# VCISwang/STCD

Measured on AMD Instinct MI355X. Metric: image-pairs/sec (256x256 bf16 SiamUnet_diff train), higher is better.
Workload: dtype bf16; 1 GPU; SiamUnet_diff(3,2) 256x256 full training step (fwd + cross_entropy + bwd + AdamW), 16 pairs/GPU, synthetic LEVIR-CD-shaped pairs resident in HBM; global_batch=16, image=256, parallelism=dp1

## Files before the change

stcd_amd/csrc/common.h:

```cpp
#pragma once
#include <hip/hip_runtime.h>
#include <stdint.h>
#include <stdio.h>
#include <string>
#include <string.h>

#include "../../include/stcd_hip.h"

namespace stcd {

typedef __bf16 bf16;

enum DType { F32 = STCD_DTYPE_F32, BF16 = STCD_DTYPE_BF16 };
inline size_t dsize(int dt) { return dt == BF16 ? 2 : 4; }

void set_error(const std::string& msg);

#define STCD_CHECK(cond, msg)                                              \
    do {                                                                   \
        if (!(cond)) {                                                     \
            ::stcd::set_error(std::string(__func__) + ": " + (msg));       \
            return 1;                                                      \
        }                                                                  \
    } while (0)
// ... 226 lines not shown
int launch_conv_halo(const stcd_conv_geom& g, const ConvMfmaPlan& p, const ConvHaloPlan& hp, const void* in, const void* wf,
                     const float* bias, void* out, hipStream_t s, const ConvEpi* epi = nullptr);

struct ConvDmaPlan {
    int tiles_m = 0, tiles_n = 0, blocks = 0, lds_bytes = 0;
    bool ok = false;
};
ConvDmaPlan conv_dma_plan(const stcd_conv_geom& g, const ConvMfmaPlan& p);
int launch_conv_dma(const stcd_conv_geom& g, const ConvMfmaPlan& p, const ConvDmaPlan& dp, const void* in, const void* wf,
                    const float* bias, void* out, hipStream_t s, const ConvEpi* epi = nullptr);

bool conv_small_ok(const stcd_conv_geom& g, const ConvMfmaPlan& p);
int conv_small_blocks(const stcd_conv_geom& g, int groups);
int launch_conv_small(const stcd_conv_geom& g, const void* in, const void* wf_modeB, const float* bias, void* out,
                      bool out_nchw_f32, int groups, long long* stat_acc, int cpad, hipStream_t s, const XfSrc* xf = nullptr,
                      const BwdSum* bs = nullptr);
bool conv_small_bwdsum_ok(const stcd_conv_geom& g);
struct WgradMfmaPlan {
    int WCI = 1, NTW = 1, gx = 1, gy = 1, gz = 1;
    int64_t slab_floats = 0;
    int wi_valid = 0;
    int gemm = 0;
    int dma = 0;
    bool ok = false;
};
WgradMfmaPlan wgrad_mfma_plan(const stcd_conv_geom& g, int kpad, int wld, bool allow_wide = false, int force_co64 = -1);
int launch_wgrad_mfma(const stcd_conv_geom& g, const WgradMfmaPlan& p, const void* in, const void* dout, float* slab,
                      int kpad, int wld, hipStream_t s);
struct WgradJob {
    stcd_conv_geom g;
    int64_t in_off, dout_off, slab_off;
    int kpad, wld;
    int dymin, dxmin, HH, HWp;
    int tiles_x, tiles_y, ntiles;
    int xrow_bytes;
    int x_bytes, y_bytes;
    int co_valid;
    unsigned in_bytes, dout_bytes;
    int gx, gy, gz;
    int start;
    int lds_bytes;
    int wi_valid;
    int dma_L, dma_nk;
    int pad_;
    int64_t xf_stat_off, xf_mask_off;
    int xf_C, xf_groups, xf_npg, pad2_;
};
WgradMfmaPlan wgrad_gemm_plan(const stcd_conv_geom& g, int kpad, int wld);
WgradJob wgrad_gemm_make_job(const stcd_conv_geom& g, const WgradMfmaPlan& p, int64_t in_off, int64_t dout_off, int64_t slab_off,
                             int kpad, int wld);
int launch_wgrad_gemm_group(int W, const WgradJob* jobs_dev, int njobs, int total_blocks, const char* base, hipStream_t s);
WgradMfmaPlan wgrad_dma_plan(const stcd_conv_geom& g, int kpad, int wld);
void wgrad_dma_set_split(WgradMfmaPlan& p, const stcd_conv_geom& g, int S, int kpad, int wld);
WgradJob wgrad_dma_make_job(const stcd_conv_geom& g, const WgradMfmaPlan& p, int64_t in_off, int64_t dout_off, int64_t slab_off,
                            int kpad, int wld);
int launch_wgrad_dma_group(const WgradJob* jobs_dev, int njobs, int total_blocks, const char* base, hipStream_t s);
WgradJob wgrad_make_job(const stcd_conv_geom& g, const WgradMfmaPlan& p, int64_t in_off, int64_t dout_off, int64_t slab_off,
                        int kpad, int wld);
void wgrad_job_set_xf(WgradJob& a, int64_t stat_off, int64_t mask_off, int C, int groups, int npg);
int wgrad_variant_slots(int WCI, int NTW, bool t9, int lds_bytes);
int launch_wgrad_group(int WCI, int NTW, bool t9, const WgradJob* jobs_dev, int njobs, int total_blocks, int lds_bytes,
                       const char* base, hipStream_t s, bool xf = false);
struct PackSpec;
struct ReduceJob {
    int64_t start, count;
    int64_t slab_off;
    int64_t out_off;
    int64_t slab_stride;
    int gx, ntaps, K, N, kpad, wld;
    int ks, kn_major;
    int8_t ky[9], kx[9];
    int8_t tiled, parts, pad_[4];
};
void launch_reduce_jobs(const ReduceJob* jobs_dev, int njobs, int64_t total, const char* ws, float* grads, hipStream_t s);
void launch_reduce_dw(const float* slab, int gx, const stcd_conv_geom& g, int K, int N, int kpad, int wld,
                      const PackSpec* ps, float* out, hipStream_t s);

struct PackSpec {
    int ks;
// ... 227 lines not shown
```

stcd_amd/csrc/engine.hip:

```cpp
#include <algorithm>
#include <climits>
#include <cstdint>
#include <array>
#include <cstring>
#include <memory>
#include <vector>

#include "common.h"

namespace stcd {

static thread_local std::string g_err;
void set_error(const std::string& msg) { g_err = msg; }

enum ConvKind { K_CONV3 = 0, K_CONVT3_S1 = 1, K_UPCONV = 2, K_CONV1 = 3, K_CONVT2 = 4, K_CONV3_S2 = 5, K_CONV1_S2 = 6, K_STEM7 = 7 };

struct TRef { int64_t off = -1; int ld = 0; };
struct GRef { int64_t off = -1; int ld = 0; int64_t goff = 0; };

static inline int round8(int c) { return (c + 7) & ~7; }

struct ConvW {
    std::string name;
    int kind = 0, cin = 0, cout = 0;
// ... 23 lines not shown
    ConvDmaPlan dma;
    ConvHaloPlan halo;
};
struct WgradOp {
    stcd_conv_geom g{};
    int conv = -1, tap0 = 0, kreal = 0, nreal = 0;
    WgradMfmaPlan plan;
    int64_t slab = -1;
    int stage = 0;
    int64_t in_off = -1, dout_off = -1;
    bool grouped = false;
    int group = -1;
    int64_t xf_stat_off = -1, xf_mask_off = -1; int xf_C = 0, xf_groups = 1, xf_npg = 1;
    bool tail = false;
    bool own_taps = false;
    int8_t oky[9] = {0}, okx[9] = {0};
};
struct WgradGroup {
    int WCI = 1, NTW = 1; bool t9 = false;
    bool xf = false;
    bool tail = false;
    int gemm = 0;
    int dma = 0;
    std::vector<WgradJob> jobs;
    int total_blocks = 0, lds_bytes = 0;
    int64_t table_off = -1;
    double flops = 0.0, bytes = 0.0;
    int seen = 0; bool launched = false;
};

struct Cbrd {
    ConvOp fwd, dgr; WgradOp wg;
    int conv = -1, bn = -1, drop = -1;
    int N = 0, H = 0, W = 0, groups = 1, npg = 0;
    TRef in; int K = 0;
    TRef Y; GRef A; TRef P; TRef dPool; bool pool = false;
    GRef dA; TRef dY; TRef dIn; bool has_dIn = false;
    int64_t stat = -1;
    int64_t facc = -1, bacc = -1;
    const Cbrd* dgr_bwd = nullptr;
    bool bwd_sums_fused = false;
    int64_t dgr_sum_acc = -1; int dgr_sum_c0 = 0, dgr_sum_C = 0;
    TRef fuse_dst;
    bool virt = false; const Cbrd* xsrc = nullptr;
};
struct XConc {
// ... 393 lines not shown
    g.ntaps = t;
    static const int start[4] = {0, 1, 3, 5};
    *tap0 = start[py * 2 + px];
    return g;
}

static void conv_work(const stcd_engine& e, const stcd_conv_geom& g, int kreal, int nreal, double* flops, double* bytes);

static void pick_gemm_or_res(const stcd_engine& e, ConvOp& op, const stcd_conv_geom& g, int groups) {
    op.gemm = ConvGemmPlan();
    if (!e.use_gemm || op.small) return;
    static const int env_mode = [] { const char* v = getenv("STCD_GEMM_OVER_RES"); return v ? atoi(v) : -1; }();
    const int mode = env_mode >= 0 ? env_mode : (e.cf ? 1 : 0);
    if (op.res.ok && !(mode == 2 || (mode == 1 && op.res.NT == 1))) return;
    op.gemm = conv_gemm_plan(g, op.plan, groups);
    if (op.gemm.ok) op.res = ConvResPlan();
    static const bool halo_on = [] { const char* v = getenv("STCD_HALO_KERNEL"); return v && v[0] == '1'; }();
    op.halo = ConvHaloPlan();
    op.dma = ConvDmaPlan();
    if (op.gemm.ok && (int64_t)g.n * g.hm * g.wm >= 256 * 192) op.dma = conv_dma_plan(g, op.plan);
    if (halo_on && op.gemm.ok && (int64_t)g.n * ((g.hm + 15) / 16) * ((g.wm + 15) / 16) >= 512) op.halo = conv_halo_plan(g, op.plan);
}

static WgradMfmaPlan pick_wgrad_plan(const stcd_engine& e, const stcd_conv_geom& g, int kpad, int wld) {
    if (e.use_gemm && e.use_wgroup && 2.0 * g.n * g.hm * g.wm * (double)g.ci * g.co >= 0.8e9) {
        WgradMfmaPlan p = wgrad_gemm_plan(g, kpad, wld);
        if (p.ok) return p;
    }
    if (e.use_wgroup && (g.ntaps == 9 || (e.cf && g.ntaps == 4)) && (int64_t)g.n * g.hm * g.wm >= 65536) {
        WgradMfmaPlan p = wgrad_dma_plan(g, kpad, wld);
        if (p.ok) return p;
    }
    return wgrad_mfma_plan(g, kpad, wld, is_snunet(e.arch) || (e.cf && g.ntaps == 9));
}

static void build_pack_jobs(stcd_engine& e, Bump& ws) {
    for (int st = 0; st < 2; ++st) { e.rjobs[st].clear(); e.rjobs_total[st] = 0; }
    for (int st = 0; st < 2; ++st) e.wgroups[st].clear();
    if (e.dt == BF16 && e.use_mfma) {
        if (e.use_wgroup) {
            for (WgradOp* op : e.wgrad_ops) {
                if (!op->plan.ok) continue;
                const bool t9 = !op->plan.dma && op->g.ntaps == 9;
                std::vector<WgradGroup>& gs = e.wgroups[op->stage];
                size_t gi = 0;
                for (; gi < gs.size(); ++gi)
                    if (gs[gi].gemm == op->plan.gemm && gs[gi].dma == op->plan.dma && gs[gi].WCI == op->plan.WCI && gs[gi].NTW == op->plan.NTW && gs[gi].t9 == t9 && gs[gi].xf == (op->xf_C > 0) && gs[gi].tail == op->tail) break;
                if (gi == gs.size()) { WgradGroup g; g.WCI = op->plan.WCI; g.NTW = op->plan.NTW; g.t9 = t9; g.gemm = op->plan.gemm; g.dma = op->plan.dma; g.xf = op->xf_C > 0; g.tail = op->tail; gs.push_back(g); }
                op->grouped = true;
            }
            for (int st = 0; st < 2; ++st)
                for (WgradGroup& G : e.wgroups[st]) {
                    if (G.gemm) { G.lds_bytes = 2 * 2 * G.gemm * (64 * 64 + 8 * 32); continue; }
                    if (G.dma) {
                        G.lds_bytes = 128 * 1024;
                        std::vector<WgradOp*> dops;
                        for (WgradOp* op : e.wgrad_ops)
                            if (op->grouped && op->stage == st && op->plan.dma) dops.push_back(op);
                        auto blocks_at = [&](int64_t kt) {
                            int64_t b = 0;
                            for (WgradOp* op : dops) {
                                const int64_t M = (int64_t)op->g.n * op->g.hi * op->g.wi;
                                b += ((M + kt * 64 - 1) / (kt * 64)) * op->plan.gy * op->plan.gz;
                            }
                            return b;
                        };
                        int64_t lo = 1, hi = 1;
                        static const int dma_env = [] { const char* v = getenv("STCD_WGRAD_DMA_BLOCKS"); return v && atoi(v) > 0 ? atoi(v) : 0; }();
                        static const bool cf_side_env = [] { const char* v = getenv("STCD_CF_SIDE"); return !(v && v[0] == '0'); }();
                        const int dma_blocks = dma_env ? dma_env : (e.wg_side_on && cf_side_env ? 192 : 256);
                        while (blocks_at(hi) > dma_blocks) hi *= 2;
                        while (lo < hi) { const int64_t mid = (lo + hi) / 2; if (blocks_at(mid) <= dma_blocks) hi = mid; else lo = mid + 1; }
                        for (WgradOp* op : dops) {
                            const ConvW& cv = e.convs[op->conv];
                            const int64_t M = (int64_t)op->g.n * op->g.hi * op->g.wi;
                            int64_t S = (M + lo * 64 - 1) / (lo * 64);
                            const int64_t slab_bytes = (int64_t)op->g.ntaps * cv.fwd.kpad * cv.fwd.wld * 4;
                            S = std::min<int64_t>(S, std::max<int64_t>(1, ((int64_t)64 << 20) / slab_bytes));
                            wgrad_dma_set_split(op->plan, op->g, (int)S, cv.fwd.kpad, cv.fwd.wld);
                        }
                        continue;
                    }
                    std::vector<WgradOp*> ops;
                    int64_t W = 0;
                    for (WgradOp* op : e.wgrad_ops)
                        if (op->grouped && op->stage == st && !op->plan.gemm && !op->plan.dma && op->plan.WCI == G.WCI && op->plan.NTW == G.NTW && (op->g.ntaps == 9) == G.t9 && (op->xf_C > 0) == G.xf && op->tail == G.tail) {
                            ops.push_back(op);
                            const int64_t ntiles = (int64_t)op->g.n * ((op->g.wm + 15) / 16) * ((op->g.hm + 7) / 8);
                            W += ntiles * op->plan.gy * op->plan.gz;
                        }
                    for (WgradOp* op : ops) {
                        const ConvW& cv = e.convs[op->conv];
                        WgradJob j = wgrad_make_job(op->g, op->plan, 0, 0, 0, cv.fwd.kpad, cv.fwd.wld);
                        if (op->xf_C > 0) wgrad_job_set_xf(j, op->xf_stat_off, op->xf_mask_off, op->xf_C, op->xf_groups, op->xf_npg);
                        G.lds_bytes = std::max(G.lds_bytes, j.lds_bytes);
                    }
                    int slots = wgrad_variant_slots(G.WCI, G.NTW, G.t9, G.lds_bytes);
                    if (st == 0 && e.wg_side_on && e.wg_side_div > 1 && fc_family(e)) slots = std::max(64, slots / e.wg_side_div);
                    const int64_t rounds = e.wgroup_rounds;
                    const int64_t tpb = std::max<int64_t>(e.wgroup_min_tiles, (W + rounds * slots - 1) / (rounds * slots));
                    for (WgradOp* op : ops) {
                        const ConvW& cv = e.convs[op->conv];
                        const int64_t ntiles = (int64_t)op->g.n * ((op->g.wm + 15) / 16) * ((op->g.hm + 7) / 8);
                        const int64_t slab_bytes = (int64_t)op->g.ntaps * cv.fwd.kpad * cv.fwd.wld * 4;
                        int64_t gx = std::max<int64_t>(1, (ntiles + tpb - 1) / tpb);
                        gx = std::min<int64_t>(gx, std::max<int64_t>(1, ((int64_t)32 << 20) / slab_bytes));
                        op->plan.gx = (int)gx;
                        op->plan.slab_floats = gx * op->g.ntaps * cv.fwd.kpad * cv.fwd.wld;
                    }
                }
        }
        int64_t cur[2] = {0, 0};
        for (WgradOp* op : e.wgrad_ops) {
            if (!op->plan.ok) continue;
            const ConvW& cv = e.convs[op->conv];
            op->slab = ws.take(op->plan.slab_floats * 4);
            if (op->grouped) {
                const bool t9 = !op->plan.dma && op->g.ntaps == 9;
                for (WgradGroup& G : e.wgroups[op->stage])
                    if (G.gemm == op->plan.gemm && G.dma == op->plan.dma && G.WCI == op->plan.WCI && G.NTW == op->plan.NTW && G.t9 == t9 && G.xf == (op->xf_C > 0) && G.tail == op->tail) {
                        op->group = (int)(&G - e.wgroups[op->stage].data());
                        WgradJob j = op->plan.dma ? wgrad_dma_make_job(op->g, op->plan, op->in_off, op->dout_off, op->slab, cv.fwd.kpad, cv.fwd.wld)
                                   : op->plan.gemm ? wgrad_gemm_make_job(op->g, op->plan, op->in_off, op->dout_off, op->slab, cv.fwd.kpad, cv.fwd.wld)
                                                   : wgrad_make_job(op->g, op->plan, op->in_off, op->dout_off, op->slab, cv.fwd.kpad, cv.fwd.wld);
                        if (op->xf_C > 0 && !op->plan.dma && !op->plan.gemm) wgrad_job_set_xf(j, op->xf_stat_off, op->xf_mask_off, op->xf_C, op->xf_groups, op->xf_npg);
                        j.start = G.total_blocks;
                        G.total_blocks += j.gx * j.gy * j.gz;
                        G.jobs.push_back(j);
                        double fl, by;
                        conv_work(e, op->g, op->kreal, op->nreal, &fl, &by);
                        G.flops += fl; G.bytes += by;
                    }
            }
            ReduceJob j{};
            j.slab_off = op->slab; j.out_off = cv.w_off;
            j.slab_stride = (int64_t)op->g.ntaps * cv.fwd.kpad * cv.fwd.wld;
            j.gx = op->plan.gx; j.ntaps = op->g.ntaps; j.K = cv.cin; j.N = cv.cout; j.kpad = cv.fwd.kpad; j.wld = cv.fwd.wld;
            j.ks = cv.fwd.ks; j.kn_major = cv.fwd.kn_major;
            for (int t = 0; t < op->g.ntaps; ++t) {
                j.ky[t] = op->own_taps ? op->oky[t] : cv.fwd.ky[op->tap0 + t];
                j.kx[t] = op->own_taps ? op->okx[t] : cv.fwd.kx[op->tap0 + t];
            }
            j.tiled = (int64_t)j.ntaps * j.K * j.N >= 512 * 1024;
            if (!j.tiled) {
                const int64_t outs = (int64_t)j.ntaps * j.K * j.N;
                int parts = 1;
                while (parts < 64 && parts * 32 < j.gx) parts *= 2;
                j.parts = (int8_t)parts;
// ... 292 lines not shown
                   (P.groups == 1 || P.dA.goff == (int64_t)P.npg * P.H * P.W * P.dA.ld);
        };
        auto scan = [&](std::vector<Cbrd>& v) {
            for (size_t i = 1; i < v.size(); ++i) {
                Cbrd& N = v[i]; Cbrd& P = v[i - 1];
                if (N.has_dIn && N.dgr_sum_acc < 0 && dest_ok(P, N.dgr, N.dIn.off, N.dIn.ld, N.N)) { N.dgr_bwd = &P; P.bwd_sums_fused = true; }
            }
        };
        scan(e.enc); scan(e.dec);
        if (!e.dec.empty() && dest_ok(e.dec.back(), e.final_dgr, e.dFinalIn.off, e.dFinalIn.ld, e.dec.back().N)) {
            e.final_dgr_bwd = &e.dec.back(); e.dec.back().bwd_sums_fused = true;
        }
    }

    e.final_xsrc = nullptr; e.fc_virt_layers = 0;
    for (auto& L : e.enc) { L.virt = false; L.xsrc = nullptr; }
    for (auto& L : e.dec) { L.virt = false; L.xsrc = nullptr; }
    if (e.use_virt && e.dt == BF16 && e.use_mfma && e.use_wgroup && !fc_cross(e)) {
        auto fwd_ok = [&](const ConvOp& op, bool nchw) {
            if (op.wf < 0 || (op.gemm.ok && !nchw)) return false;
            if (op.small && e.use_small) return true;
            return op.res.ok && !nchw && !op.res.single_halo;
        };
        auto wg_ok = [&](const WgradOp& op) { return op.plan.ok && !op.plan.gemm && !op.plan.dma && op.plan.WCI < 4 && op.plan.NTW < 4; };
        auto link = [&](Cbrd& P, ConvOp& cf, WgradOp& cw, bool nchw) {
            if (P.pool || P.fuse_dst.off >= 0) return false;
            if (!fwd_ok(cf, nchw) || !wg_ok(cw)) return false;
            P.virt = true; ++e.fc_virt_layers;
            cw.in_off = P.Y.off;
            cw.xf_stat_off = P.stat;
            cw.xf_mask_off = (P.drop >= 0) ? e.masks + e.drops[P.drop].off * 4 : -1;
            cw.xf_C = e.convs[P.conv].cout; cw.xf_groups = P.groups; cw.xf_npg = P.npg;
            return true;
        };
        for (size_t i = 0; i + 1 < e.enc.size(); ++i) {
            Cbrd& P = e.enc[i]; Cbrd& Cn = e.enc[i + 1];
            if (Cn.in.off != P.A.off) continue;
            if (link(P, Cn.fwd, Cn.wg, false)) { Cn.xsrc = &P; Cn.in.off = P.Y.off; Cn.in.ld = P.Y.ld; }
        }
        for (size_t i = 0; i < e.dec.size(); ++i) {
            Cbrd& P = e.dec[i];
            if (i + 1 < e.dec.size() && e.dec[i + 1].in.off == P.A.off) {
                Cbrd& Cn = e.dec[i + 1];
                if (link(P, Cn.fwd, Cn.wg, false)) { Cn.xsrc = &P; Cn.in.off = P.Y.off; Cn.in.ld = P.Y.ld; }
            } else if (e.finalIn.off == P.A.off) {
                if (link(P, e.final_fwd, e.final_wg, true)) { e.final_xsrc = &P; e.finalIn.off = P.Y.off; e.finalIn.ld = P.Y.ld; }
            }
        }
    }

// ... 234 lines not shown
                                        hipMemcpyHostToDevice, c.s));
            if (!e.rjobs[k].empty())
                STCD_HIP(hipMemcpyAsync(c.at(e.rjobs_off[k]), e.rjobs[k].data(), e.rjobs[k].size() * sizeof(ReduceJob),
                                        hipMemcpyHostToDevice, c.s));
            for (WgradGroup& G : e.wgroups[k])
                STCD_HIP(hipMemcpyAsync(c.at(G.table_off), G.jobs.data(), G.jobs.size() * sizeof(WgradJob), hipMemcpyHostToDevice, c.s));
        }
        if (!e.bias_jobs.empty())
            STCD_HIP(hipMemcpyAsync(c.at(e.bias_jobs_off), e.bias_jobs.data(), e.bias_jobs.size() * sizeof(BiasJob), hipMemcpyHostToDevice, c.s));
        e.jobs_uploaded_ws = c.ws;
    }
    const int k = with_dgrad ? 1 : 0;
    if (k == 0 && e.weights_tag != 0 && e.weights_tag == e.packed_tag && e.packed_ws == (const void*)c.ws && e.packed_params == (const void*)c.params)
        return 0;
    ProfScope prof(c, PC_PACK, 0.0, 0.0);
    launch_pack_jobs(c.at<PackJob>(e.jobs_off[k]), (int)e.jobs[k].size(), e.jobs_total[k], c.params, c.ws, c.s);
    e.packed_tag = k == 0 ? e.weights_tag : 0; e.packed_ws = c.ws; e.packed_params = c.params; e.packed_level = k;
    return 0;
}

static void launch_wgroup(const Ctx& c, WgradGroup& G) {
    {
        char kname[64];
        if (G.dma) snprintf(kname, sizeof(kname), "k_wgrad_dma");
        else if (G.gemm) snprintf(kname, sizeof(kname), "k_wgrad_gemm<%d>", G.gemm);
        else snprintf(kname, sizeof(kname), "k_wgrad_group<%d, %d, %s>", G.WCI, G.NTW, G.t9 ? "true" : "false");
        ProfScope prof(c, PC_WGRAD, G.flops, G.bytes, kname);
        G.launched = true;
        if (G.dma) {
            launch_wgrad_dma_group(c.at<WgradJob>(G.table_off), (int)G.jobs.size(), G.total_blocks, c.ws, c.s);
            return;
        }
        if (G.gemm) {
            launch_wgrad_gemm_group(G.gemm, c.at<WgradJob>(G.table_off), (int)G.jobs.size(), G.total_blocks, c.ws, c.s);
            return;
        }
        if (launch_wgrad_group(G.WCI, G.NTW, G.t9, c.at<WgradJob>(G.table_off), (int)G.jobs.size(), G.total_blocks, G.lds_bytes,
                               c.ws, c.s, G.xf) != 0)
            set_error("grouped weight-gradient launch exceeds the LDS budget");
    }
}

static void wgroup_member_ready(const Ctx& c, const WgradOp& op) {
    stcd_engine& e = c.e;
    if (op.group < 0 || op.group >= (int)e.wgroups[op.stage].size()) return;
    WgradGroup& G = e.wgroups[op.stage][op.group];
    if (++G.seen < (int)G.jobs.size() || G.launched) return;
    if (e.wg_cur_side) {
        if (hipEventRecord(e.wg_fork, c.s) != hipSuccess || hipStreamWaitEvent(e.wg_cur_side, e.wg_fork, 0) != hipSuccess) { set_error("side-stream fork failed"); return; }
        Ctx cs{e, c.ws, c.params, c.grads, e.wg_cur_side};
        launch_wgroup(cs, G);
// ... 1935 lines not shown
}

static int check_geom(const stcd_conv_geom* g) {
    STCD_CHECK(g != nullptr, "geometry is null");
    STCD_CHECK(g->ntaps >= 1 && g->ntaps <= 9, "ntaps must be in [1,9]");
    STCD_CHECK(g->ci >= 8 && g->ci % 8 == 0 && g->ldi >= g->ci && g->ldi % 8 == 0, "ci/ldi must be multiples of 8");
    STCD_CHECK(g->co >= 1 && g->ldo >= g->co, "bad co/ldo");
    STCD_CHECK(g->in_stride >= 1 && g->out_stride >= 1 && g->n >= 1 && g->hm >= 1 && g->wm >= 1, "bad sizes");
    STCD_CHECK((g->hm - 1) * g->out_stride + g->oy0 < g->ho && (g->wm - 1) * g->out_stride + g->ox0 < g->wo,
               "output positions exceed the output buffer");
    return 0;
}
static int op_dma_splits(const stcd_conv_geom& g, const WgradMfmaPlan& p) {
    const int64_t M = (int64_t)g.n * g.hi * g.wi;
    return (int)std::max<int64_t>(1, std::min<int64_t>(256 / std::max(1, p.gy * p.gz), M / 512));
}
int64_t stcd_op_scratch_bytes(const stcd_conv_geom* g) {
    if (!g) return 0;
    ConvMfmaPlan p = conv_mfma_plan(*g);
    WgradMfmaPlan w = wgrad_mfma_plan(*g, g->ci, g->co), ww = wgrad_mfma_plan(*g, g->ci, g->co, true);
    WgradMfmaPlan wg = wgrad_gemm_plan(*g, g->ci, g->co);
    WgradMfmaPlan wd = wgrad_dma_plan(*g, g->ci, g->co);
    if (wd.ok) wgrad_dma_set_split(wd, *g, op_dma_splits(*g, wd), g->ci, g->co);
    return std::max<int64_t>(p.wf_elems * 2, std::max(std::max(std::max(w.slab_floats, ww.slab_floats), wg.ok ? wg.slab_floats : 0), wd.ok ? wd.slab_floats : 0) * 4) + 1024;
}
int stcd_op_conv(int dtype, int impl, const stcd_conv_geom* g, const void* in, const float* w, const float* bias,
                 void* out, void* scratch, int64_t scratch_bytes, void* hip_stream) {
    if (check_geom(g)) return 1;
    STCD_CHECK(in && w && out, "null pointer argument");
    if (impl == 1 || impl == 2 || impl == 3 || impl == 6) {
        STCD_CHECK(dtype == STCD_DTYPE_BF16, "the MFMA implementation is bf16 only");
        ConvMfmaPlan p = conv_mfma_plan(*g);
        STCD_CHECK(p.ok, "geometry not supported by the MFMA kernel");
        STCD_CHECK(scratch && scratch_bytes >= p.wf_elems * 2, "scratch too small for the fragment-order filter");
        launch_pack_frag(*g, p, w, g->ci, g->co, scratch, (hipStream_t)hip_stream);
        if (impl == 3) {
            const ConvHaloPlan hp = conv_halo_plan(*g, p);
            STCD_CHECK(hp.ok, "geometry not supported by the resident-halo kernel (3x3 stride 1, Ci % 64 == 0, Co % 128 == 0)");
            STCD_CHECK(launch_conv_halo(*g, p, hp, in, scratch, bias, out, (hipStream_t)hip_stream) == 0, "launch failed");
            STCD_HIP(hipGetLastError());
            return 0;
        }
        if (impl == 6) {
            const ConvDmaPlan dp = conv_dma_plan(*g, p);
            STCD_CHECK(dp.ok, "geometry not supported by the LDS-DMA kernel (Ci % 64 == 0, Co % 256 == 0, (Ci / 64) * taps even and >= 4)");
            STCD_CHECK(launch_conv_dma(*g, p, dp, in, scratch, bias, out, (hipStream_t)hip_stream) == 0, "launch failed");
            STCD_HIP(hipGetLastError());
// ... 37 lines not shown
        WgradMfmaPlan p = wgrad_mfma_plan(*g, g->ci, g->co, impl >= 4, impl == 5 ? 1 : 0);
        STCD_CHECK(p.ok, "geometry not supported by the MFMA kernel");
        STCD_CHECK(scratch && scratch_bytes >= p.slab_floats * 4, "scratch too small for the partial slabs");
        STCD_CHECK(launch_wgrad_mfma(*g, p, in, dout, (float*)scratch, g->ci, g->co, (hipStream_t)hip_stream) == 0, "LDS budget exceeded");
        launch_reduce_dw((const float*)scratch, p.gx, *g, g->ci, g->co, g->ci, g->co, nullptr, dw, (hipStream_t)hip_stream);
        STCD_HIP(hipGetLastError());
        return 0;
    }
    if (impl == 7) {
        STCD_CHECK(dtype == STCD_DTYPE_BF16, "the MFMA implementation is bf16 only");
        WgradMfmaPlan p = wgrad_dma_plan(*g, g->ci, g->co);
        STCD_CHECK(p.ok, "geometry not supported by the LDS-DMA weight-gradient kernel (stride 1, full map >= 64 wide, Ci % 256 == 0, Co % 256 == 0)");
        wgrad_dma_set_split(p, *g, op_dma_splits(*g, p), g->ci, g->co);
        const int64_t table = (p.slab_floats * 4 + 255) & ~(int64_t)255;
        STCD_CHECK(scratch && scratch_bytes >= table + (int64_t)sizeof(WgradJob), "scratch too small for the partial slabs + job table");
        WgradJob j = wgrad_dma_make_job(*g, p, (int64_t)(intptr_t)in, (int64_t)(intptr_t)dout, (int64_t)(intptr_t)scratch, g->ci, g->co);
        STCD_HIP(hipMemcpyAsync((char*)scratch + table, &j, sizeof(j), hipMemcpyHostToDevice, (hipStream_t)hip_stream));
        STCD_HIP(hipStreamSynchronize((hipStream_t)hip_stream));
        launch_wgrad_dma_group((const WgradJob*)((char*)scratch + table), 1, p.gx * p.gy * p.gz, nullptr, (hipStream_t)hip_stream);
        launch_reduce_dw((const float*)scratch, p.gx, *g, g->ci, g->co, g->ci, g->co, nullptr, dw, (hipStream_t)hip_stream);
        STCD_HIP(hipGetLastError());
        return 0;
    }
    if (impl == 3) {
        STCD_CHECK(dtype == STCD_DTYPE_BF16, "the MFMA implementation is bf16 only");
        WgradMfmaPlan p = wgrad_gemm_plan(*g, g->ci, g->co);
        STCD_CHECK(p.ok, "geometry not supported by the GEMM weight-gradient kernel (one tap, Ci >= 64, Co >= 64)");
        const int64_t table = (p.slab_floats * 4 + 255) & ~(int64_t)255;
        STCD_CHECK(scratch && scratch_bytes >= table + (int64_t)sizeof(WgradJob), "scratch too small for the partial slabs + job table");
        WgradJob j = wgrad_gemm_make_job(*g, p, (int64_t)(intptr_t)in, (int64_t)(intptr_t)dout, (int64_t)(intptr_t)scratch, g->ci, g->co);
        STCD_HIP(hipMemcpyAsync((char*)scratch + table, &j, sizeof(j), hipMemcpyHostToDevice, (hipStream_t)hip_stream));
        STCD_HIP(hipStreamSynchronize((hipStream_t)hip_stream));
        launch_wgrad_gemm_group(p.gemm, (const WgradJob*)((char*)scratch + table), 1, p.gx * p.gy * p.gz, nullptr, (hipStream_t)hip_stream);
        launch_reduce_dw((const float*)scratch, p.gx, *g, g->ci, g->co, g->ci, g->co, nullptr, dw, (hipStream_t)hip_stream);
        STCD_HIP(hipGetLastError());
        return 0;
    }
    STCD_CHECK(impl == 0, "impl must be 0 (reference FMA), 1 / 4 (MFMA tile kernel, 4: wide tile allowed), 3 (MFMA position-GEMM kernel) or 7 (LDS-DMA kernel)");
    STCD_HIP(hipMemsetAsync(dw, 0, (size_t)g->ntaps * g->ci * g->co * 4, (hipStream_t)hip_stream));
    launch_wgrad_ref(dtype, *g, in, dout, dw, g->ci, g->co, (hipStream_t)hip_stream);
    STCD_HIP(hipGetLastError());
    return 0;
}

}
```

Before: 7772 image-pairs/sec.

## Add row-streaming MFMA weight-gradient kernel for narrow-channel 3x3 convs

Adds a new weight-gradient kernel that streams whole image rows of input and output-gradient through LDS ring buffers with buffer-to-LDS DMA. It computes all nine 3x3 taps from three resident input rows using transposed LDS reads and bf16 MFMA, then reduces partial slabs across blocks. The planner uses it for large-map convs with few channels (Ci 8-32, Co <=32) in the SiamUnet family, splitting a fixed block budget across grouped ops in proportion to their size. The aim is to cut redundant input reloads and the poor MFMA utilisation of the tile kernel on thin channels. In exchange it uses a large LDS footprint with one block per CU, and it falls back to the tile plan when the layer is fused with a virtual forward.

```diff
diff --git a/stcd_amd/csrc/common.h b/stcd_amd/csrc/common.h
--- a/stcd_amd/csrc/common.h
+++ b/stcd_amd/csrc/common.h
@@ -272,6 +272,7 @@
     int wi_valid = 0;
     int gemm = 0;
     int dma = 0;
+    int rows = 0;
     bool ok = false;
 };
 WgradMfmaPlan wgrad_mfma_plan(const stcd_conv_geom& g, int kpad, int wld, bool allow_wide = false, int force_co64 = -1);
@@ -305,6 +306,11 @@
 WgradJob wgrad_dma_make_job(const stcd_conv_geom& g, const WgradMfmaPlan& p, int64_t in_off, int64_t dout_off, int64_t slab_off,
                             int kpad, int wld);
 int launch_wgrad_dma_group(const WgradJob* jobs_dev, int njobs, int total_blocks, const char* base, hipStream_t s);
+WgradMfmaPlan wgrad_rows_plan(const stcd_conv_geom& g, int kpad, int wld, bool force = false);
+void wgrad_rows_set_blocks(WgradMfmaPlan& p, const stcd_conv_geom& g, int blocks, int kpad, int wld);
+WgradJob wgrad_rows_make_job(const stcd_conv_geom& g, const WgradMfmaPlan& p, int64_t in_off, int64_t dout_off, int64_t slab_off,
+                             int kpad, int wld);
+int launch_wgrad_rows_group(const WgradJob* jobs_dev, int njobs, int total_blocks, int lds_bytes, const char* base, hipStream_t s);
 WgradJob wgrad_make_job(const stcd_conv_geom& g, const WgradMfmaPlan& p, int64_t in_off, int64_t dout_off, int64_t slab_off,
                         int kpad, int wld);
 void wgrad_job_set_xf(WgradJob& a, int64_t stat_off, int64_t mask_off, int C, int groups, int npg);
diff --git a/stcd_amd/csrc/engine.hip b/stcd_amd/csrc/engine.hip
--- a/stcd_amd/csrc/engine.hip
+++ b/stcd_amd/csrc/engine.hip
@@ -69,6 +69,7 @@
     bool tail = false;
     int gemm = 0;
     int dma = 0;
+    int rows = 0;
     std::vector<WgradJob> jobs;
     int total_blocks = 0, lds_bytes = 0;
     int64_t table_off = -1;
@@ -508,6 +509,9 @@
     if (halo_on && op.gemm.ok && (int64_t)g.n * ((g.hm + 15) / 16) * ((g.wm + 15) / 16) >= 512) op.halo = conv_halo_plan(g, op.plan);
 }
 
+static WgradMfmaPlan wgrad_tile_plan(const stcd_engine& e, const stcd_conv_geom& g, int kpad, int wld) {
+    return wgrad_mfma_plan(g, kpad, wld, is_snunet(e.arch) || (e.cf && g.ntaps == 9));
+}
 static WgradMfmaPlan pick_wgrad_plan(const stcd_engine& e, const stcd_conv_geom& g, int kpad, int wld) {
     if (e.use_gemm && e.use_wgroup && 2.0 * g.n * g.hm * g.wm * (double)g.ci * g.co >= 0.8e9) {
         WgradMfmaPlan p = wgrad_gemm_plan(g, kpad, wld);
@@ -517,7 +521,11 @@
         WgradMfmaPlan p = wgrad_dma_plan(g, kpad, wld);
         if (p.ok) return p;
     }
-    return wgrad_mfma_plan(g, kpad, wld, is_snunet(e.arch) || (e.cf && g.ntaps == 9));
+    if (e.use_wgroup && e.use_mfma && fc_family(e) && (int64_t)g.n * g.hm * g.wm >= 65536) {
+        WgradMfmaPlan p = wgrad_rows_plan(g, kpad, wld);
+        if (p.ok && p.WCI * p.NTW > 1) return p;
+    }
+    return wgrad_tile_plan(e, g, kpad, wld);
 }
 
 static void build_pack_jobs(stcd_engine& e, Bump& ws) {
@@ -531,8 +539,8 @@
                 std::vector<WgradGroup>& gs = e.wgroups[op->stage];
                 size_t gi = 0;
                 for (; gi < gs.size(); ++gi)
-                    if (gs[gi].gemm == op->plan.gemm && gs[gi].dma == op->plan.dma && gs[gi].WCI == op->plan.WCI && gs[gi].NTW == op->plan.NTW && gs[gi].t9 == t9 && gs[gi].xf == (op->xf_C > 0) && gs[gi].tail == op->tail) break;
-                if (gi == gs.size()) { WgradGroup g; g.WCI = op->plan.WCI; g.NTW = op->plan.NTW; g.t9 = t9; g.gemm = op->plan.gemm; g.dma = op->plan.dma; g.xf = op->xf_C > 0; g.tail = op->tail; gs.push_back(g); }
+                    if (gs[gi].gemm == op->plan.gemm && gs[gi].dma == op->plan.dma && gs[gi].rows == op->plan.rows && gs[gi].WCI == op->plan.WCI && gs[gi].NTW == op->plan.NTW && gs[gi].t9 == t9 && gs[gi].xf == (op->xf_C > 0) && gs[gi].tail == op->tail) break;
+                if (gi == gs.size()) { WgradGroup g; g.WCI = op->plan.WCI; g.NTW = op->plan.NTW; g.t9 = t9; g.gemm = op->plan.gemm; g.dma = op->plan.dma; g.rows = op->plan.rows; g.xf = op->xf_C > 0; g.tail = op->tail; gs.push_back(g); }
                 op->grouped = true;
             }
             for (int st = 0; st < 2; ++st)
@@ -567,10 +575,27 @@
                         }
                         continue;
                     }
+                    if (G.rows) {
+                        std::vector<WgradOp*> rops;
+                        double total = 0.0;
+                        for (WgradOp* op : e.wgrad_ops)
+                            if (op->grouped && op->stage == st && op->plan.rows && op->plan.WCI == G.WCI && op->plan.NTW == G.NTW && op->tail == G.tail) {
+                                rops.push_back(op);
+                                total += (double)op->g.n * op->g.hi * op->g.wi * (op->g.ci + op->g.co);
+                            }
+                        for (WgradOp* op : rops) {
+                            const ConvW& cv = e.convs[op->conv];
+                            const double share = (double)op->g.n * op->g.hi * op->g.wi * (op->g.ci + op->g.co) / total;
+                            wgrad_rows_set_blocks(op->plan, op->g, std::max(1, (int)(256 * share + 0.5)), cv.fwd.kpad, cv.fwd.wld);
+                            const WgradJob j = wgrad_rows_make_job(op->g, op->plan, 0, 0, 0, cv.fwd.kpad, cv.fwd.wld);
+                            G.lds_bytes = std::max(G.lds_bytes, j.lds_bytes);
+                        }
+                        continue;
+                    }
                     std::vector<WgradOp*> ops;
                     int64_t W = 0;
                     for (WgradOp* op : e.wgrad_ops)
-                        if (op->grouped && op->stage == st && !op->plan.gemm && !op->plan.dma && op->plan.WCI == G.WCI && op->plan.NTW == G.NTW && (op->g.ntaps == 9) == G.t9 && (op->xf_C > 0) == G.xf && op->tail == G.tail) {
+                        if (op->grouped && op->stage == st && !op->plan.gemm && !op->plan.dma && !op->plan.rows && op->plan.WCI == G.WCI && op->plan.NTW == G.NTW && (op->g.ntaps == 9) == G.t9 && (op->xf_C > 0) == G.xf && op->tail == G.tail) {
                             ops.push_back(op);
                             const int64_t ntiles = (int64_t)op->g.n * ((op->g.wm + 15) / 16) * ((op->g.hm + 7) / 8);
                             W += ntiles * op->plan.gy * op->plan.gz;
@@ -604,12 +629,13 @@
             if (op->grouped) {
                 const bool t9 = !op->plan.dma && op->g.ntaps == 9;
                 for (WgradGroup& G : e.wgroups[op->stage])
-                    if (G.gemm == op->plan.gemm && G.dma == op->plan.dma && G.WCI == op->plan.WCI && G.NTW == op->plan.NTW && G.t9 == t9 && G.xf == (op->xf_C > 0) && G.tail == op->tail) {
+                    if (G.gemm == op->plan.gemm && G.dma == op->plan.dma && G.rows == op->plan.rows && G.WCI == op->plan.WCI && G.NTW == op->plan.NTW && G.t9 == t9 && G.xf == (op->xf_C > 0) && G.tail == op->tail) {
                         op->group = (int)(&G - e.wgroups[op->stage].data());
-                        WgradJob j = op->plan.dma ? wgrad_dma_make_job(op->g, op->plan, op->in_off, op->dout_off, op->slab, cv.fwd.kpad, cv.fwd.wld)
+                        WgradJob j = op->plan.rows ? wgrad_rows_make_job(op->g, op->plan, op->in_off, op->dout_off, op->slab, cv.fwd.kpad, cv.fwd.wld)
+                                   : op->plan.dma ? wgrad_dma_make_job(op->g, op->plan, op->in_off, op->dout_off, op->slab, cv.fwd.kpad, cv.fwd.wld)
                                    : op->plan.gemm ? wgrad_gemm_make_job(op->g, op->plan, op->in_off, op->dout_off, op->slab, cv.fwd.kpad, cv.fwd.wld)
                                                    : wgrad_make_job(op->g, op->plan, op->in_off, op->dout_off, op->slab, cv.fwd.kpad, cv.fwd.wld);
-                        if (op->xf_C > 0 && !op->plan.dma && !op->plan.gemm) wgrad_job_set_xf(j, op->xf_stat_off, op->xf_mask_off, op->xf_C, op->xf_groups, op->xf_npg);
+                        if (op->xf_C > 0 && !op->plan.dma && !op->plan.gemm && !op->plan.rows) wgrad_job_set_xf(j, op->xf_stat_off, op->xf_mask_off, op->xf_C, op->xf_groups, op->xf_npg);
                         j.start = G.total_blocks;
                         G.total_blocks += j.gx * j.gy * j.gz;
                         G.jobs.push_back(j);
@@ -948,10 +974,12 @@
             if (op.small && e.use_small) return true;
             return op.res.ok && !nchw && !op.res.single_halo;
         };
-        auto wg_ok = [&](const WgradOp& op) { return op.plan.ok && !op.plan.gemm && !op.plan.dma && op.plan.WCI < 4 && op.plan.NTW < 4; };
+        auto wg_ok = [&](const WgradMfmaPlan& pl) { return pl.ok && !pl.gemm && !pl.dma && !pl.rows && pl.WCI < 4 && pl.NTW < 4; };
         auto link = [&](Cbrd& P, ConvOp& cf, WgradOp& cw, bool nchw) {
             if (P.pool || P.fuse_dst.off >= 0) return false;
-            if (!fwd_ok(cf, nchw) || !wg_ok(cw)) return false;
+            const WgradMfmaPlan pl = cw.plan.rows ? wgrad_tile_plan(e, cw.g, e.convs[cw.conv].fwd.kpad, e.convs[cw.conv].fwd.wld) : cw.plan;
+            if (!fwd_ok(cf, nchw) || !wg_ok(pl)) return false;
+            cw.plan = pl;
             P.virt = true; ++e.fc_virt_layers;
             cw.in_off = P.Y.off;
             cw.xf_stat_off = P.stat;
@@ -1232,11 +1260,17 @@
 static void launch_wgroup(const Ctx& c, WgradGroup& G) {
     {
         char kname[64];
-        if (G.dma) snprintf(kname, sizeof(kname), "k_wgrad_dma");
+        if (G.rows) snprintf(kname, sizeof(kname), "k_wgrad_rows");
+        else if (G.dma) snprintf(kname, sizeof(kname), "k_wgrad_dma");
         else if (G.gemm) snprintf(kname, sizeof(kname), "k_wgrad_gemm<%d>", G.gemm);
         else snprintf(kname, sizeof(kname), "k_wgrad_group<%d, %d, %s>", G.WCI, G.NTW, G.t9 ? "true" : "false");
         ProfScope prof(c, PC_WGRAD, G.flops, G.bytes, kname);
         G.launched = true;
+        if (G.rows) {
+            if (launch_wgrad_rows_group(c.at<WgradJob>(G.table_off), (int)G.jobs.size(), G.total_blocks, G.lds_bytes, c.ws, c.s) != 0)
+                set_error("grouped weight-gradient launch exceeds the LDS budget");
+            return;
+        }
         if (G.dma) {
             launch_wgrad_dma_group(c.at<WgradJob>(G.table_off), (int)G.jobs.size(), G.total_blocks, c.ws, c.s);
             return;
@@ -3218,7 +3252,8 @@
     WgradMfmaPlan wg = wgrad_gemm_plan(*g, g->ci, g->co);
     WgradMfmaPlan wd = wgrad_dma_plan(*g, g->ci, g->co);
     if (wd.ok) wgrad_dma_set_split(wd, *g, op_dma_splits(*g, wd), g->ci, g->co);
-    return std::max<int64_t>(p.wf_elems * 2, std::max(std::max(std::max(w.slab_floats, ww.slab_floats), wg.ok ? wg.slab_floats : 0), wd.ok ? wd.slab_floats : 0) * 4) + 1024;
+    WgradMfmaPlan wr = wgrad_rows_plan(*g, g->ci, g->co, true);
+    return std::max<int64_t>(p.wf_elems * 2, std::max(std::max(std::max(std::max(w.slab_floats, ww.slab_floats), wg.ok ? wg.slab_floats : 0), wd.ok ? wd.slab_floats : 0), wr.ok ? wr.slab_floats : 0) * 4) + 1024;
 }
 int stcd_op_conv(int dtype, int impl, const stcd_conv_geom* g, const void* in, const float* w, const float* bias,
                  void* out, void* scratch, int64_t scratch_bytes, void* hip_stream) {
@@ -3302,6 +3337,20 @@
         STCD_HIP(hipGetLastError());
         return 0;
     }
+    if (impl == 8) {
+        STCD_CHECK(dtype == STCD_DTYPE_BF16, "the MFMA implementation is bf16 only");
+        WgradMfmaPlan p = wgrad_rows_plan(*g, g->ci, g->co, true);
+        STCD_CHECK(p.ok, "geometry not supported by the row-streaming weight-gradient kernel (3x3 stride 1, full map, Ci in {8, 16, 24, 32}, Co <= 32, plain X)");
+        const int64_t table = (p.slab_floats * 4 + 255) & ~(int64_t)255;
+        STCD_CHECK(scratch && scratch_bytes >= table + (int64_t)sizeof(WgradJob), "scratch too small for the partial slabs + job table");
+        WgradJob j = wgrad_rows_make_job(*g, p, (int64_t)(intptr_t)in, (int64_t)(intptr_t)dout, (int64_t)(intptr_t)scratch, g->ci, g->co);
+        STCD_HIP(hipMemcpyAsync((char*)scratch + table, &j, sizeof(j), hipMemcpyHostToDevice, (hipStream_t)hip_stream));
+        STCD_HIP(hipStreamSynchronize((hipStream_t)hip_stream));
+        STCD_CHECK(launch_wgrad_rows_group((const WgradJob*)((char*)scratch + table), 1, p.gx, j.lds_bytes, nullptr, (hipStream_t)hip_stream) == 0, "LDS budget exceeded");
+        launch_reduce_dw((const float*)scratch, p.gx, *g, g->ci, g->co, g->ci, g->co, nullptr, dw, (hipStream_t)hip_stream);
+        STCD_HIP(hipGetLastError());
+        return 0;
+    }
     if (impl == 3) {
         STCD_CHECK(dtype == STCD_DTYPE_BF16, "the MFMA implementation is bf16 only");
         WgradMfmaPlan p = wgrad_gemm_plan(*g, g->ci, g->co);
@@ -3316,7 +3365,7 @@
         STCD_HIP(hipGetLastError());
         return 0;
     }
-    STCD_CHECK(impl == 0, "impl must be 0 (reference FMA), 1 / 4 (MFMA tile kernel, 4: wide tile allowed), 3 (MFMA position-GEMM kernel) or 7 (LDS-DMA kernel)");
+    STCD_CHECK(impl == 0, "impl must be 0 (reference FMA), 1 / 4 (MFMA tile kernel, 4: wide tile allowed), 3 (MFMA position-GEMM kernel), 7 (LDS-DMA kernel) or 8 (row-streaming kernel)");
     STCD_HIP(hipMemsetAsync(dw, 0, (size_t)g->ntaps * g->ci * g->co * 4, (hipStream_t)hip_stream));
     launch_wgrad_ref(dtype, *g, in, dout, dw, g->ci, g->co, (hipStream_t)hip_stream);
     STCD_HIP(hipGetLastError());
diff --git a/stcd_amd/csrc/kernels_wgrad_rows.hip b/stcd_amd/csrc/kernels_wgrad_rows.hip
--- /dev/null
+++ b/stcd_amd/csrc/kernels_wgrad_rows.hip
@@ -0,0 +1,330 @@
+#include <algorithm>
+#include <cstdlib>
+
+#include "common.h"
+
+namespace stcd {
+
+typedef __attribute__((ext_vector_type(8))) __bf16 bf16x8;
+typedef __attribute__((ext_vector_type(4))) __bf16 bf16x4;
+typedef __attribute__((ext_vector_type(4))) float f32x4;
+
+constexpr int WR_XSLOTS = 6, WR_YSLOTS = 4;
+constexpr int WR_MAXPW = 8;
+constexpr unsigned WR_OOB = 0x80000000u;
+#define WR_LDS(P_) ((__attribute__((address_space(3))) void*)(P_))
+
+template <int T>
+__device__ __forceinline__ int wr_phys(int p, int c) {
+    if constexpr (T == 1) return (p ^ (((p >> 3) & 1) << 2)) * 32 + c * 16;
+    else return p * 64 + ((c ^ (((p >> 3) & 1) << 1)) * 16);
+}
+
+__device__ __forceinline__ bf16x4 wr_tr(unsigned addr) {
+    bf16x4 v;
+    asm volatile("ds_read_b64_tr_b16 %0, %1" : "=v"(v) : "v"(addr) : "memory");
+    return v;
+}
+__device__ __forceinline__ bf16x8 wr_cat(bf16x4 lo, bf16x4 hi) {
+    bf16x8 f;
+    f[0] = lo[0]; f[1] = lo[1]; f[2] = lo[2]; f[3] = lo[3];
+    f[4] = hi[0]; f[5] = hi[1]; f[6] = hi[2]; f[7] = hi[3];
+    return f;
+}
+
+#define WR_BAR()                                                                                                       \
+    do {                                                                                                               \
+        __builtin_amdgcn_sched_barrier(0);                                                                             \
+        __builtin_amdgcn_s_barrier();                                                                                  \
+        __builtin_amdgcn_sched_barrier(0);                                                                             \
+    } while (0)
+#define WR_LGKM(N_)                                                                                                    \
+    do {                                                                                                               \
+        asm volatile("s_waitcnt lgkmcnt(" #N_ ")" ::: "memory");                                                       \
+        __builtin_amdgcn_sched_barrier(0);                                                                             \
+    } while (0)
+
+template <int CIT, int COT>
+__device__ __forceinline__ void wgrad_rows_body(const WgradJob& a, const char* base, const int blk) {
+    extern __shared__ __attribute__((aligned(16))) char smem[];
+    constexpr int NP = CIT * COT, WK = 4 / NP;
+    constexpr int PBX = 32 * CIT, PBY = 32 * COT;
+    const int tid = threadIdx.x, lane = tid & 63;
+    const int wid = __builtin_amdgcn_readfirstlane(tid >> 6);
+    const int pair = wid % NP, wk = wid / NP, tci = pair % CIT, tco = pair / CIT;
+    const int grp = lane >> 4, li = lane & 15, qrow = li >> 2, pcol = li & 3;
+    const int W = a.g.wi, H = a.g.hi, NH = a.ntiles, ldi = a.g.ldi, ldo = a.g.ldo;
+    const int nks = a.tiles_x;
+    const int XS = a.x_bytes, YS = a.y_bytes, NX = XS >> 10, NY = YS >> 10, PW = a.dma_nk;
+    const int r0 = min(NH, blk * a.dma_L), r1 = min(NH, r0 + a.dma_L), nrows = r1 - r0;
+    const int zrow_off = WR_XSLOTS * XS, yring_off = (WR_XSLOTS + 1) * XS, dummy_off = yring_off + WR_YSLOTS * YS;
+
+    const __amdgpu_buffer_rsrc_t xrs = __builtin_amdgcn_make_buffer_rsrc(
+        const_cast<char*>(base + a.in_off), (short)0, (int)a.in_bytes, 0x00020000);
+    const __amdgpu_buffer_rsrc_t yrs = __builtin_amdgcn_make_buffer_rsrc(
+        const_cast<char*>(base + a.dout_off), (short)0, (int)a.dout_bytes, 0x00020000);
+    const int xrow_b = W * ldi * 2, yrow_b = W * ldo * 2;
+
+    unsigned voff[WR_MAXPW];
+#pragma unroll
+    for (int ii = 0; ii < WR_MAXPW; ++ii) {
+        const int g = wid + 4 * ii;
+        unsigned v = WR_OOB;
+        if (g < NX) {
+            const int P = g * 64 + lane;
+            int p, c;
+            if constexpr (CIT == 1) { const int pp = P >> 1; p = pp ^ (((pp >> 3) & 1) << 2); c = P & 1; }
+            else { p = P >> 2; c = (P & 3) ^ (((p >> 3) & 1) << 1); }
+            const int x = p - 1;
+            if (x >= 0 && x < W && c * 8 < a.g.ci) v = (unsigned)((x * ldi + c * 8) * 2);
+        } else if (g < NX + NY) {
+            const int P = (g - NX) * 64 + lane;
+            int p, c;
+            if constexpr (COT == 1) { const int pp = P >> 1; p = pp ^ (((pp >> 3) & 1) << 2); c = P & 1; }
+            else { p = P >> 2; c = (P & 3) ^ (((p >> 3) & 1) << 1); }
+            if (p < W && c * 8 < a.co_valid) v = (unsigned)((p * ldo + c * 8) * 2);
+        }
+        voff[ii] = v;
+    }
+#define WR_STAGE(S_, XSLOT_, YSLOT_)                                                                                   \
+    do {                                                                                                               \
+        const int rx_ = r0 + (S_) + 1, ry_ = r0 + (S_);                                                                \
+        const bool xok_ = rx_ >= 0 && rx_ <= r1 && rx_ < NH;                                                           \
+        const bool yok_ = (S_) >= 0 && ry_ < r1;                                                                       \
+        const int xso_ = xok_ ? rx_ * xrow_b : 0, yso_ = yok_ ? ry_ * yrow_b : 0;                                      \
+        const int xdst_ = (XSLOT_) * XS, ydst_ = yring_off + (YSLOT_) * YS;                                            \
+        _Pragma("unroll") for (int ii = 0; ii < WR_MAXPW; ++ii) {                                                      \
+            if (ii < PW) {                                                                                             \
+                const int g_ = wid + 4 * ii;                                                                           \
+                if (g_ < NX) {                                                                                         \
+                    __builtin_amdgcn_raw_ptr_buffer_load_lds(xrs, WR_LDS(smem + xdst_ + g_ * 1024), 16,                \
+                                                             (int)(xok_ ? voff[ii] : WR_OOB), xso_, 0, 0);             \
+                } else if (g_ < NX + NY && (S_) >= 0) {                                                                \
+                    __builtin_amdgcn_raw_ptr_buffer_load_lds(yrs, WR_LDS(smem + ydst_ + (g_ - NX) * 1024), 16,         \
+                                                             (int)(yok_ ? voff[ii] : WR_OOB), yso_, 0, 0);             \
+                } else {                                                                                               \
+                    __builtin_amdgcn_raw_ptr_buffer_load_lds(xrs, WR_LDS(smem + dummy_off), 16, (int)WR_OOB, 0, 0, 0); \
+                }                                                                                                      \
+            }                                                                                                          \
+        }                                                                                                              \
+    } while (0)
+#define WR_WAIT2()                                                                                                     \
+    do {                                                                                                               \
+        switch (PW) {                                                                                                  \
+            case 1: asm volatile("s_waitcnt vmcnt(2)" ::: "memory"); break;                                            \
+            case 2: asm volatile("s_waitcnt vmcnt(4)" ::: "memory"); break;                                            \
+            case 3: asm volatile("s_waitcnt vmcnt(6)" ::: "memory"); break;                                            \
+            case 4: asm volatile("s_waitcnt vmcnt(8)" ::: "memory"); break;                                            \
+            case 5: asm volatile("s_waitcnt vmcnt(10)" ::: "memory"); break;                                           \
+            case 6: asm volatile("s_waitcnt vmcnt(12)" ::: "memory"); break;                                           \
+            case 7: asm volatile("s_waitcnt vmcnt(14)" ::: "memory"); break;                                           \
+            default: asm volatile("s_waitcnt vmcnt(16)" ::: "memory"); break;                                          \
+        }                                                                                                              \
+    } while (0)
+
+    const unsigned lds0 = (unsigned)(uintptr_t)(__attribute__((address_space(3))) char*)smem;
+    unsigned xlo[3][2], ylo[2];
+#pragma unroll
+    for (int h = 0; h < 2; ++h) {
+        const int kk = 8 * grp + qrow + 4 * h;
+        ylo[h] = lds0 + (unsigned)(wr_phys<COT>(kk, tco * 2 + (pcol >> 1)) + (pcol & 1) * 8);
+#pragma unroll
+        for (int d = 0; d < 3; ++d)
+            xlo[d][h] = lds0 + (unsigned)(wr_phys<CIT>(kk + d, tci * 2 + (pcol >> 1)) + (pcol & 1) * 8);
+    }
+
+    f32x4 acc[9];
+#pragma unroll
+    for (int t = 0; t < 9; ++t) acc[t] = f32x4{0.f, 0.f, 0.f, 0.f};
+
+    for (int g = wid; g < NX; g += 4)
+        __builtin_amdgcn_raw_ptr_buffer_load_lds(xrs, WR_LDS(smem + zrow_off + g * 1024), 16, (int)WR_OOB, 0, 0, 0);
+    WR_STAGE(-2, 0, 0);
+    WR_STAGE(-1, 1, 0);
+    WR_STAGE(0, 2, 0);
+    WR_STAGE(1, 3, 1);
+    WR_STAGE(2, 4, 2);
+    int xslot = 0, yslot = 0;
+    int y = r0 % H;
+    for (int j = 0; j < nrows; ++j) {
+        WR_WAIT2();
+        WR_BAR();
+        {
+            int xn = xslot + 5; if (xn >= WR_XSLOTS) xn -= WR_XSLOTS;
+            int yn = yslot + 3; if (yn >= WR_YSLOTS) yn -= WR_YSLOTS;
+            WR_STAGE(j + 3, xn, yn);
+        }
+        __builtin_amdgcn_sched_barrier(0);
+        unsigned xrow[3];
+#pragma unroll
+        for (int d = 0; d < 3; ++d) {
+            int sl = xslot + d; if (sl >= WR_XSLOTS) sl -= WR_XSLOTS;
+            const bool in = (unsigned)(y + d - 1) < (unsigned)H;
+            xrow[d] = (unsigned)(in ? sl * XS : zrow_off);
+        }
+        const unsigned yrow = (unsigned)(yring_off + yslot * YS);
+        for (int ks = wk; ks < nks; ks += WK) {
+            const unsigned ya = yrow + (unsigned)(ks * 32 * PBY);
+            const unsigned xk = (unsigned)(ks * 32 * PBX);
+            bf16x4 l0[3], h0[3], l1[3], h1[3], l2[3], h2[3];
+            const bf16x4 yl = wr_tr(ylo[0] + ya), yh = wr_tr(ylo[1] + ya);
+#pragma unroll
+            for (int d = 0; d < 3; ++d) { l0[d] = wr_tr(xlo[d][0] + xrow[0] + xk); h0[d] = wr_tr(xlo[d][1] + xrow[0] + xk); }
+#pragma unroll
+            for (int d = 0; d < 3; ++d) { l1[d] = wr_tr(xlo[d][0] + xrow[1] + xk); h1[d] = wr_tr(xlo[d][1] + xrow[1] + xk); }
+            WR_LGKM(6);
+            const bf16x8 yf = wr_cat(yl, yh);
+#pragma unroll
+            for (int d = 0; d < 3; ++d)
+                acc[d] = __builtin_amdgcn_mfma_f32_16x16x32_bf16(wr_cat(l0[d], h0[d]), yf, acc[d], 0, 0, 0);
+            __builtin_amdgcn_sched_barrier(0);
+#pragma unroll
+            for (int d = 0; d < 3; ++d) { l2[d] = wr_tr(xlo[d][0] + xrow[2] + xk); h2[d] = wr_tr(xlo[d][1] + xrow[2] + xk); }
+            WR_LGKM(6);
+#pragma unroll
+            for (int d = 0; d < 3; ++d)
+                acc[3 + d] = __builtin_amdgcn_mfma_f32_16x16x32_bf16(wr_cat(l1[d], h1[d]), yf, acc[3 + d], 0, 0, 0);
+            __builtin_amdgcn_sched_barrier(0);
+            WR_LGKM(0);
+#pragma unroll
+            for (int d = 0; d < 3; ++d)
+                acc[6 + d] = __builtin_amdgcn_mfma_f32_16x16x32_bf16(wr_cat(l2[d], h2[d]), yf, acc[6 + d], 0, 0, 0);
+            __builtin_amdgcn_sched_barrier(0);
+        }
+        if (++xslot == WR_XSLOTS) xslot = 0;
+        if (++yslot == WR_YSLOTS) yslot = 0;
+        if (++y == H) y = 0;
+    }
+    asm volatile("s_waitcnt vmcnt(0)" ::: "memory");
+    __syncthreads();
+#undef WR_STAGE
+#undef WR_WAIT2
+
+    float* red = reinterpret_cast<float*>(smem);
+    constexpr int PERW = 9 * 4 * 64;
+    if (wk > 0) {
+        float* dst = red + ((wk - 1) * NP + pair) * PERW + lane;
+#pragma unroll
+        for (int t = 0; t < 9; ++t)
+#pragma unroll
+            for (int j = 0; j < 4; ++j) dst[(t * 4 + j) * 64] = acc[t][j];
+    }
+    __syncthreads();
+    if (wk == 0) {
+#pragma unroll 1
+        for (int w = 1; w < WK; ++w) {
+            const float* src = red + ((w - 1) * NP + pair) * PERW + lane;
+#pragma unroll
+            for (int t = 0; t < 9; ++t)
+#pragma unroll
+                for (int j = 0; j < 4; ++j) acc[t][j] += src[(t * 4 + j) * 64];
+        }
+        float* slab = reinterpret_cast<float*>(const_cast<char*>(base) + a.slab_off) + (int64_t)blk * 9 * a.kpad * a.wld;
+        const int co = tco * 16 + li;
+#pragma unroll
+        for (int t = 0; t < 9; ++t) {
+            int ts = 0;
+            for (int u = 0; u < 9; ++u)
+                if (a.g.dy[u] == t / 3 - 1 && a.g.dx[u] == t % 3 - 1) ts = u;
+#pragma unroll
+            for (int j = 0; j < 4; ++j) {
+                const int ci = tci * 16 + 4 * grp + j;
+                if (ci < a.kpad && co < a.wld) slab[((int64_t)ts * a.kpad + ci) * a.wld + co] = acc[t][j];
+            }
+        }
+    }
+}
+
+__global__ void __launch_bounds__(256, 1)
+k_wgrad_rows(const WgradJob* __restrict__ jobs, int njobs, const char* base) {
+    int lo = 0, hi = njobs - 1;
+    while (lo < hi) {
+        const int mid = (lo + hi + 1) >> 1;
+        if (jobs[mid].start <= (int)blockIdx.x) lo = mid; else hi = mid - 1;
+    }
+    const WgradJob& a = jobs[lo];
+    const int blk = blockIdx.x - a.start;
+    const int cit = a.g.ci > 16 ? 2 : 1, cot = a.g.co > 16 ? 2 : 1;
+    if (cit == 1 && cot == 1) wgrad_rows_body<1, 1>(a, base, blk);
+    else if (cit == 1) wgrad_rows_body<1, 2>(a, base, blk);
+    else if (cot == 1) wgrad_rows_body<2, 1>(a, base, blk);
+    else wgrad_rows_body<2, 2>(a, base, blk);
+}
+
+static bool wgrad_rows_enabled() {
+    const char* e = getenv("STCD_NO_WGRAD_ROWS");
+    return !(e && e[0] == '1');
+}
+
+static void wgrad_rows_sizes(const stcd_conv_geom& g, int* xs, int* ys, int* pw, int* lds) {
+    const int cit = g.ci > 16 ? 2 : 1, cot = g.co > 16 ? 2 : 1, np = cit * cot;
+    const int wr = (g.wi + 31) / 32 * 32;
+    *xs = ((wr + 8) * 32 * cit + 1023) / 1024 * 1024;
+    *ys = (wr * 32 * cot + 1023) / 1024 * 1024;
+    *pw = ((*xs + *ys) / 1024 + 3) / 4;
+    *lds = std::max((WR_XSLOTS + 1) * *xs + WR_YSLOTS * *ys + 1024, (4 / np - 1) * np * 9 * 4 * 64 * 4);
+}
+
+WgradMfmaPlan wgrad_rows_plan(const stcd_conv_geom& g, int kpad, int wld, bool force) {
+    WgradMfmaPlan p;
+    if (!force && !wgrad_rows_enabled()) return p;
+    if (g.ntaps != 9 || g.in_stride != 1 || g.out_stride != 1 || g.hm != g.hi || g.wm != g.wi || g.ho != g.hi || g.wo != g.wi ||
+        g.oy0 != 0 || g.ox0 != 0) return p;
+    if (g.ci < 8 || g.ci > 32 || g.ci % 8 != 0 || g.co < 1 || g.co > 32 || g.ldi % 8 != 0 || g.ldo % 8 != 0 || g.ldi < g.ci ||
+        g.ldo < ((g.co + 7) & ~7)) return p;
+    unsigned seen = 0;
+    for (int t = 0; t < 9; ++t) {
+        if (g.dy[t] < -1 || g.dy[t] > 1 || g.dx[t] < -1 || g.dx[t] > 1) return p;
+        seen |= 1u << ((g.dy[t] + 1) * 3 + g.dx[t] + 1);
+    }
+    if (seen != 0x1ffu) return p;
+    if ((int64_t)g.n * g.hi * g.wi * g.ldi * 2 >= ((int64_t)1 << 31) || (int64_t)g.n * g.hi * g.wi * g.ldo * 2 >= ((int64_t)1 << 31)) return p;
+    int xs, ys, pw, lds;
+    wgrad_rows_sizes(g, &xs, &ys, &pw, &lds);
+    if (pw > WR_MAXPW || lds > 160 * 1024) return p;
+    p.rows = 1;
+    p.WCI = g.ci > 16 ? 2 : 1; p.NTW = g.co > 16 ? 2 : 1;
+    p.gy = 1; p.gz = 1;
+    p.ok = true;
+    wgrad_rows_set_blocks(p, g, 256, kpad, wld);
+    return p;
+}
+
+void wgrad_rows_set_blocks(WgradMfmaPlan& p, const stcd_conv_geom& g, int blocks, int kpad, int wld) {
+    const int64_t NH = (int64_t)g.n * g.hi;
+    const int64_t B = std::max<int64_t>(1, std::min<int64_t>(blocks, NH));
+    const int64_t L = (NH + B - 1) / B;
+    p.gx = (int)((NH + L - 1) / L);
+    p.slab_floats = (int64_t)p.gx * 9 * kpad * wld;
+}
+
+WgradJob wgrad_rows_make_job(const stcd_conv_geom& g, const WgradMfmaPlan& p, int64_t in_off, int64_t dout_off, int64_t slab_off,
+                             int kpad, int wld) {
+    WgradJob a;
+    memset(&a, 0, sizeof(a));
+    a.g = g;
+    a.in_off = in_off; a.dout_off = dout_off; a.slab_off = slab_off; a.kpad = kpad; a.wld = wld;
+    const int64_t NH = (int64_t)g.n * g.hi;
+    a.ntiles = (int)NH;
+    a.tiles_x = (g.wi + 31) / 32;
+    a.dma_L = (int)((NH + p.gx - 1) / p.gx);
+    wgrad_rows_sizes(g, &a.x_bytes, &a.y_bytes, &a.dma_nk, &a.lds_bytes);
+    a.co_valid = (g.co + 7) & ~7;
+    a.in_bytes = (unsigned)(NH * g.wi * g.ldi * 2);
+    a.dout_bytes = (unsigned)(NH * g.wi * g.ldo * 2);
+    a.gx = p.gx; a.gy = 1; a.gz = 1; a.start = 0;
+    a.wi_valid = g.wi;
+    a.xf_stat_off = -1; a.xf_mask_off = -1; a.xf_groups = 1; a.xf_npg = 1;
+    return a;
+}
+
+int launch_wgrad_rows_group(const WgradJob* jobs_dev, int njobs, int total_blocks, int lds_bytes, const char* base, hipStream_t s) {
+    if (njobs <= 0 || total_blocks <= 0) return 0;
+    if (lds_bytes > 160 * 1024) return 1;
+    static bool attr_set = false;
+    if (!attr_set) { (void)hipFuncSetAttribute((const void*)k_wgrad_rows, hipFuncAttributeMaxDynamicSharedMemorySize, 160 * 1024); attr_set = true; }
+    k_wgrad_rows<<<(unsigned)total_blocks, 256, (size_t)lds_bytes, s>>>(jobs_dev, njobs, base);
+    return 0;
+}
+
+}
```

After: 7638 image-pairs/sec. 0.983x the previous value.
